# neuromodulation/py_neuromodulation

Hardware: AMD Instinct MI355X
Metric: windows/sec (all features), 256 ch @ 1 kHz (higher is better)
Workload: dtype f32; 1 GPU; 256ch/GPU @1kHz, W=1000, hop=100, 1024 hops/step, all 9 hot-path features, 4 bands, notch50+CAR, z-score normalisation; channels_per_gpu=256, features_per_window=9984, parallelism=channel-shard x1, no collective

## Files before the change

py_neuromodulation_amd/csrc/nmx_k_bank_w64.h:

```cpp
#pragma once

#include "nmx_k_bank.h"
#include "nmx_k_fft500.h"
#include "nmx_k_sharpwave.h"

#ifdef NMX_HOST_EMU
#define NMX_UNROLL
#else
#define NMX_UNROLL _Pragma("unroll")
#endif

#ifdef NMX_HOST_EMU
#define NMX_SCHED_FENCE() ((void)0)
#else
#define NMX_SCHED_FENCE() __builtin_amdgcn_sched_barrier(0)
#endif

#if defined(NMX_BANK_PROFILE) && !defined(NMX_HOST_EMU)
#define NMX_PROF_DECL long long pf_t = clock64(), pf_acc[8] = {0, 0, 0, 0, 0, 0, 0, 0};
#define NMX_PROF(i) { const long long t_ = clock64(); pf_acc[i] += t_ - pf_t; pf_t = t_; }
#define NMX_PROF_PRINT(w, c)                                                                                          \
  if ((w) == 5 && ((c) == 3 || (c) == 40) && (threadIdx.x & 63) == 0)                                                  \
    printf("bank profile w=%d c=%d: load+fwd %lld | spectral+passA %lld | passB load+dft %lld | passB store %lld | "  \
           "passC %lld | variance %lld | series stores %lld | partners %lld (cycles, whole item, %d filters)\n", (w), (c), pf_acc[0],   \
// ... 417 lines not shown
      }
#endif
    }
  }
  NMX_WSYNC();
  NMX_LANE_LOOP { nmx_w64_passA<-1>(v[NMX_LI], X, l); }
  NMX_WSYNC();
  NMX_LANE_LOOP { nmx_w64_passB_load_lds<-1, TAB>(v[NMX_LI], X, twB, l); }
  NMX_WSYNC();
  NMX_LANE_LOOP { nmx_w64_passB_store(v[NMX_LI], X, l); }
  NMX_WSYNC();
  NMX_LANE_LOOP {
    nmx_c2* vv = v[NMX_LI];
    nmx_w64_passC_lds<-1, TAB>(vv, X, twC, l);
    NMX_UNROLL
    for (int i = 0; i < 16; ++i) zr[NMX_LI][i] = vv[i];
  }
  NMX_WSYNC();
  NMX_PROF(0)

#ifndef NMX_HOST_EMU
  nmx_c2 zcr[16];
  if (PAD == 0) {
    const int l = (int)(threadIdx.x & 63);
    NMX_UNROLL
    for (int r = 0; r < 16; ++r) {
      const nmx_c2 zs = zr[0][NMX_J2I(15 - r)];
      nmx_c2 zc = nmx_mk2(__shfl(zs.x, (64 - l) & 63), __shfl(zs.y, (64 - l) & 63));
      if (l == 0) zc = (r == 0) ? zr[0][0] : zr[0][NMX_J2I((16 - r) & 15)];
      zcr[r] = zc;
    }
  }
#endif
  NMX_PROF(6)
  const int yoff = (PAD == 1) ? A.pad_half : 0;
  for (int fi = 0; fi < A.n_filters; ++fi) {
    const NmxFilterDev& F = A.f[fi];
    const float* NMX_RESTRICT Hs = TAB ? tab + (size_t)fi * 2 * NMX_W64_N : AA.Hs[fi];
    const float* NMX_RESTRICT Hd = TAB ? tab + (size_t)fi * 2 * NMX_W64_N + NMX_W64_N : AA.Hd[fi];
    NMX_LANE_LOOP {
      nmx_c2* vv = v[NMX_LI];
      NMX_UNROLL
      for (int r = 0; r < 16; ++r) {
        const nmx_c2 zk = zr[NMX_LI][NMX_J2I(r)];
#ifdef NMX_HOST_EMU
        nmx_c2 zc = zr[(64 - l) & 63][NMX_J2I(15 - r)];
        if (l == 0) zc = (r == 0) ? zr[NMX_LI][0] : zr[NMX_LI][NMX_J2I((16 - r) & 15)];
#else
        nmx_c2 zc;
        if (PAD == 0) {
          zc = zcr[r];
        } else {
          const nmx_c2 zs = zr[0][NMX_J2I(15 - r)];
          zc = nmx_mk2(__shfl(zs.x, (64 - l) & 63), __shfl(zs.y, (64 - l) & 63));
          if (l == 0) zc = (r == 0) ? zr[0][0] : zr[0][NMX_J2I((16 - r) & 15)];
        }
#endif
        const float ha = (Hs + l)[64 * r], hb = (Hd + l)[64 * r];
        vv[r] = nmx_c2_axpby_swap(ha, zk, hb, zc);
        if ((r & 3) == 3) NMX_SCHED_FENCE();
      }
      nmx_w64_passA<+1>(vv, X, l);
    }
    NMX_WSYNC();
    NMX_PROF(1)
    NMX_LANE_LOOP { nmx_w64_passB_load_lds<+1, TAB>(v[NMX_LI], X, twB, l); }
    NMX_WSYNC();
    NMX_PROF(2)
    NMX_LANE_LOOP { nmx_w64_passB_store(v[NMX_LI], X, l); }
    NMX_WSYNC();
    NMX_PROF(3)
    NMX_LANE_LOOP { nmx_w64_passC_lds<+1, TAB>(v[NMX_LI], X, twC, l); }
    NMX_PROF(4)

    if (F.bp_seglen > 0) {
      const bool need_mc = MC && (A.bp_features & 6u) != 0;
      if (!need_mc) {
        const int lo = W - F.bp_seglen + yoff, hi = W + yoff;
        float part[NMX_LANES], part2[NMX_LANES];
        NMX_LANE_LOOP {
          nmx_c2 acc = nmx_mk2(0.f, 0.f), acc2 = nmx_mk2(0.f, 0.f);
#if defined(NMX_HOST_EMU)
          NMX_UNROLL
          for (int i = 0; i < 16; ++i) {
            const int mb = 64 * (i >> 2) + 256 * (i & 3);
            if (2 * mb + 127 < lo || 2 * mb >= hi) continue;
            nmx_c2 val = v[NMX_LI][i];
            if (!(2 * mb >= lo && 2 * mb + 127 < hi)) val = nmx_w64_range_mask(val, l + mb, lo, hi);
            acc = nmx_cadd(acc, val);
            acc2 = nmx_c2_fma(val, val, acc2);
          }
#else
          const unsigned span = (unsigned)(hi - lo);
          const int s_l = 2 * l - lo;
          NMX_UNROLL
          for (int i = 0; i < 16; ++i) {
            const int sb = s_l + 2 * (64 * (i >> 2) + 256 * (i & 3));
            nmx_c2 val = v[NMX_LI][i];
            val.x = (unsigned)sb < span ? val.x : 0.f;
            val.y = (unsigned)(sb + 1) < span ? val.y : 0.f;
            acc = nmx_cadd(acc, val);
            acc2 = nmx_c2_fma(val, val, acc2);
          }
#endif
          part[NMX_LI] = acc.x + acc.y;
          part2[NMX_LI] = acc2.x + acc2.y;
        }
        float tot, tot2;
        NMX_W64_REDUCE_SUM(part, tot);
        NMX_W64_REDUCE_SUM(part2, tot2);
        const float mean = tot / (float)F.bp_seglen;
        tot = tot2 - mean * tot;
        if (mean * mean * (float)F.bp_seglen > 4.f * tot) {
          NMX_LANE_LOOP {
            nmx_c2 acc = nmx_mk2(0.f, 0.f);
            const nmx_c2 mean2 = nmx_mk2(mean, mean);
            NMX_UNROLL
            for (int i = 0; i < 16; ++i) {
              const int mb = 64 * (i >> 2) + 256 * (i & 3);
              if (2 * mb + 127 < lo || 2 * mb >= hi) continue;
              nmx_c2 d = nmx_csub(v[NMX_LI][i], mean2);
              if (!(2 * mb >= lo && 2 * mb + 127 < hi)) d = nmx_w64_range_mask(d, l + mb, lo, hi);
              acc = nmx_c2_fma(d, d, acc);
            }
            part[NMX_LI] = acc.x + acc.y;
          }
          NMX_W64_REDUCE_SUM(part, tot);
        }
        const float act = tot / (float)F.bp_seglen;
        NMX_LANE_LOOP {
          if (l == 0) {
            const int col = A.bp_cols.base + c * A.bp_cols.ch_stride + F.bp_band * A.bp_cols.a_stride;
            out_row[col] = nmx_bp_activity(A.bp_log ? log10f(act) : act, (A.bp_kalman_mask >> F.bp_band) & 1u);
          }
        }
      } else {
        NMX_WSYNC();
        NMX_LANE_LOOP {
          NMX_UNROLL
          for (int i = 0; i < 16; ++i) X[l + 64 * (i >> 2) + 256 * (i & 3)] = v[NMX_LI][i];
        }
        NMX_WSYNC();
        const float* y = (const float*)X + yoff;
        float act, mob, comp;
        nmx_hjorth(y + (W - F.bp_seglen), F.bp_seglen, red, 1, true, act, mob, comp);
        if (NMX_TID == 0) {
          int col = A.bp_cols.base + c * A.bp_cols.ch_stride + F.bp_band * A.bp_cols.a_stride;
          if (A.bp_features & 1u) { out_row[col] = nmx_bp_activity(A.bp_log ? log10f(act) : act, (A.bp_kalman_mask >> F.bp_band) & 1u); col += A.bp_cols.b_stride; }
          if (A.bp_features & 2u) { out_row[col] = nmx_nan_to_num(mob); col += A.bp_cols.b_stride; }
          if (A.bp_features & 4u) out_row[col] = nmx_nan_to_num(comp);
        }
      }
    }
    NMX_PROF(5)
    if (PAD == 0) {
      float* dsw = F.sw_index >= 0
          ? A.sw_out + (((long long)w * A.n_channels + c) * A.n_sw_filters + F.sw_index) * W : nullptr;
      float* dyb = F.burst_index >= 0
          ? AA.yb_out + (((long long)w * A.n_channels + c) * A.n_burst_bands + F.burst_index) * W : nullptr;
#ifdef NMX_HOST_EMU
      NMX_LANE_LOOP {
        for (int i = 0; i < 16; ++i) {
          const int m = l + 64 * (i >> 2) + 256 * (i & 3);
          const nmx_c2 val = v[NMX_LI][i];
          if (2 * m < W) { if (dsw) dsw[2 * m] = val.x; if (dyb) dyb[2 * m] = val.x; }
          if (2 * m + 1 < W) { if (dsw) dsw[2 * m + 1] = val.y; if (dyb) dyb[2 * m + 1] = val.y; }
        }
      }
#else
      const int l = (int)(threadIdx.x & 63);
      for (int dst = 0; dst < 2; ++dst) {
        float* d = dst ? dyb : dsw;
        if (!d) continue;
        const nmx_rsrc rs = nmx_make_rsrc(d, 4 * W);
        if ((W & 1) == 0) {
          NMX_UNROLL
          for (int i = 0; i < 16; ++i) {
            __builtin_amdgcn_raw_buffer_store_b64(v[0][i], rs, 8 * l + 512 * (i >> 2) + 2048 * (i & 3), 0, NMX_SERIES_STORE_AUX);
          }
        } else {
          NMX_UNROLL
          for (int i = 0; i < 16; ++i) {
            const int off = 8 * l + 512 * (i >> 2) + 2048 * (i & 3);
            __builtin_amdgcn_raw_buffer_store_b32(__float_as_uint(v[0][i].x), rs, off, 0, NMX_SERIES_STORE_AUX);
            __builtin_amdgcn_raw_buffer_store_b32(__float_as_uint(v[0][i].y), rs, off + 4, 0, NMX_SERIES_STORE_AUX);
          }
        }
      }
#endif
    } else if (F.store_raw) {
#ifndef NMX_HOST_EMU
      {
        const int l = (int)(threadIdx.x & 63);
        const nmx_rsrc rd = nmx_make_rsrc(A.y_out + ((long long)w * A.n_channels + c) * W, 4 * W);
        NMX_UNROLL
        for (int i = 0; i < 16; ++i) {
          const int s0 = 2 * (l + 64 * (i >> 2) + 256 * (i & 3)) - yoff;
          nmx_c2 val = v[0][i];
          if (A.residual) {
            const nmx_rsrc rx = nmx_make_rsrc(src, 4 * W);
            nmx_c2 xw = nmx_mk2(__uint_as_float(__builtin_amdgcn_raw_buffer_load_b32(rx, 4 * s0, 0, 0)),
                                __uint_as_float(__builtin_amdgcn_raw_buffer_load_b32(rx, 4 * s0 + 4, 0, 0)));
            if (A.clean_on_load) xw = nmx_mk2(nmx_clean_bl(xw.x), nmx_clean_bl(xw.y));
            val = xw - val;
          }
          __builtin_amdgcn_raw_buffer_store_b32(__float_as_uint(val.x), rd, 4 * s0, 0, 0);
          __builtin_amdgcn_raw_buffer_store_b32(__float_as_uint(val.y), rd, 4 * s0 + 4, 0, 0);
        }
      }
#else
      float* d2 = A.y_out + ((long long)w * A.n_channels + c) * W - yoff;
      NMX_LANE_LOOP {
        NMX_UNROLL
        for (int i = 0; i < 16; ++i) {
          const int s0 = 2 * (l + 64 * (i >> 2) + 256 * (i & 3));
          const nmx_c2 val = v[NMX_LI][i];
          if (s0 >= yoff && s0 < W + yoff)
            d2[s0] = A.residual ? (A.clean_on_load ? nmx_clean(src[s0 - yoff]) : src[s0 - yoff]) - val.x : val.x;
          if (s0 + 1 >= yoff && s0 + 1 < W + yoff)
            d2[s0 + 1] = A.residual ? (A.clean_on_load ? nmx_clean(src[s0 + 1 - yoff]) : src[s0 + 1 - yoff]) - val.y : val.y;
        }
      }
#endif
    }
    NMX_WSYNC();
    NMX_PROF(7)
  }
  NMX_PROF_PRINT(w, c)
}

struct NmxHilbertArgs {
  const float* y;
  float* env;
  int W;
  NmxFft hil_r;
  NmxFft hil_c;
  int hil_full;
  int off_a, off_b, off_y, lds_floats;
  const float* w500_tab;
  const float* w1000_tab;
  const float* floor;
  unsigned char* full;
  int n_seq, overlap;
  int long_mode, split_d, sub_m;
  const float2* tw_n;
  int slab_floats;
  int slab_blocks;
  float* slab;
};

NMX_DEV void nmx_hilbert_long_item(const NmxHilbertArgs& A, long long item, float* smem, float* slab);

NMX_DEV void nmx_hilbert_item(const NmxHilbertArgs& A, long long item, float* smem) {
  if (A.long_mode) { nmx_hilbert_long_item(A, item, smem, A.slab); return; }
  float2* bufA = (float2*)(smem + A.off_a);
  float2* bufB = (float2*)(smem + A.off_b);
  const int W = A.W, Wh = W >> 1;
  const float* src = A.y + item * W;
  float* dst = A.env + item * W;
  if (!A.hil_full) {
    float* ys = smem + A.off_y;
    float* pk = (float*)bufB;
    nmx_stage_row(src, W, [=](int i, float v) { pk[i] = v; ys[i] = v; });
    NMX_SYNC();
    const float2* Zy = nmx_fft_auto<-1, true>(A.hil_r, bufB, bufA, bufB);
    float2* Yb = (Zy == bufA) ? bufB : bufA;
    for (int k = NMX_TID; k <= Wh; k += NMX_NT) Yb[k] = nmx_rfft_bin(Zy, A.hil_r.twr, Wh, k);
    NMX_SYNC();
    float2* Pre = (Yb == bufA) ? bufB : bufA;
    for (int k = NMX_TID; k < Wh; k += NMX_NT) {
      const float2 yk = Yb[k], yn = Yb[Wh - k];
      const float2 xk = k == 0 ? make_float2(0.f, 0.f) : make_float2(yk.y, -yk.x);
      const float2 xn = k == 0 ? make_float2(0.f, 0.f) : make_float2(yn.y, -yn.x);
      Pre[k] = nmx_irfft_pre(xk, xn, A.hil_r.twr[k]);
    }
    NMX_SYNC();
    const float* ht = (const float*)nmx_fft_auto<+1, true>(A.hil_r, Pre, Yb, Pre);
    const float invW = 1.f / (float)W;
    for (int i = NMX_TID; i < W; i += NMX_NT) {
      const float re = ys[i], im = ht[i] * invW;
      dst[i] = nmx_sqrt_fast(re * re + im * im);
    }
    return;
  }
  nmx_stage_row(src, W, [=](int i, float v) { bufB[i] = make_float2(v, 0.f); });
  NMX_SYNC();
  const float2* Zy = nmx_fft_auto<-1, true>(A.hil_r, bufB, bufA, bufB);
  float2* Ab = (Zy == bufA) ? bufB : bufA;
  const float invW = 1.f / (float)W;
  for (int k = NMX_TID; k < W; k += NMX_NT) {
    float2 val = make_float2(0.f, 0.f);
    if (k == 0) val = Zy[0];
    else if (k <= (W - 1) / 2) val = make_float2(2.f * Zy[k].x, 2.f * Zy[k].y);
    Ab[k] = make_float2(val.x * invW, val.y * invW);
  }
  NMX_SYNC();
  float2* Zbuf = (Ab == bufA) ? bufB : bufA;
  const float2* an = nmx_fft_auto<+1, true>(A.hil_c, Ab, Zbuf, Ab);
  for (int i = NMX_TID; i < W; i += NMX_NT) dst[i] = nmx_sqrt_fast(an[i].x * an[i].x + an[i].y * an[i].y);
}

#ifndef NMX_HOST_EMU
#define NMX_W500_LDS_FLOATS (1008 + 1000)
template <bool SPARSE>
NMX_DEV void nmx_hilbert_w500_item(const NmxHilbertArgs& A, long long item, float* smem) {
  const int l = NMX_TID;
  nmx_c2* hb = (nmx_c2*)smem;
  nmx_c2* ha = hb + 504;
#ifdef NMX_DEBUG_HILBERT_SAMEROW
  const nmx_rsrc rin = nmx_make_rsrc(A.y + (item & 1023) * 1000, 4000);
#else
  const nmx_rsrc rin = nmx_make_rsrc(A.y + item * 1000, 4000);
#endif
  const nmx_rsrc rout = nmx_make_rsrc(A.env + item * 1000, 4000);
  const float fl = SPARSE ? A.floor[(int)item % A.n_seq] : 0.f;
  NmxW500TwReg T;
  T.load(A.w500_tab, l);
  nmx_c2 y[8];
#pragma unroll
  for (int q = 0; q < 8; ++q) y[q] = __builtin_amdgcn_raw_buffer_load_b64(rin, 8 * l + 512 * q, 0, 0);
#pragma unroll
  for (int q = 0; q < 8; ++q)
    if (q < 7 || l < 52) hb[l + 64 * q] = y[q];
  NMX_WAVE_FENCE();
  const nmx_c2* ht = nmx_w500_hilbert(ha, hb, T, (const nmx_c2*)A.w500_tab + NMX_W500_TW_N, l);
  if (SPARSE) {
    bool hit = !(fl > -INFINITY);
#pragma unroll
    for (int q = 0; q < 8; ++q) {
      const nmx_c2 h = ht[l + 64 * q];
      y[q] = nmx_mk2(nmx_sqrt_fast(y[q].x * y[q].x + h.x * h.x), nmx_sqrt_fast(y[q].y * y[q].y + h.y * h.y));
      hit = hit || ((q < 7 || l < 52) && (y[q].x >= fl || y[q].y >= fl));
    }
    const bool row = __ballot(hit) != 0ull;
    const int keep = 1000 - A.overlap;
#pragma unroll
    for (int q = 0; q < 8; ++q)
      if (row || 2 * (l + 64 * q) + 2 > keep) __builtin_amdgcn_raw_buffer_store_b64(y[q], rout, 8 * l + 512 * q, 0, 0);
    if (l == 0) A.full[item] = row ? 1 : 0;
    return;
  }
#pragma unroll
  for (int q = 0; q < 8; ++q) {
    const nmx_c2 h = ht[l + 64 * q];
    const nmx_c2 e = nmx_mk2(nmx_sqrt_fast(y[q].x * y[q].x + h.x * h.x), nmx_sqrt_fast(y[q].y * y[q].y + h.y * h.y));
    __builtin_amdgcn_raw_buffer_store_b64(e, rout, 8 * l + 512 * q, 0, 0);
  }
}
#define NMX_W1000_LDS_FLOATS 2000
template <bool SPARSE>
NMX_DEV void nmx_hilbert_w1000_item(const NmxHilbertArgs& A, long long item, float* smem) {
  const int l = NMX_TID;
  nmx_c2* hb = (nmx_c2*)smem;
  nmx_c2* ha = hb;
  const nmx_rsrc rin = nmx_make_rsrc(A.y + item * 2000, 8000);
  const nmx_rsrc rout = nmx_make_rsrc(A.env + item * 2000, 8000);
  const float fl = SPARSE ? A.floor[(int)(item % (long long)A.n_seq)] : 0.f;
  NmxW1000TwReg T;
  T.load(A.w1000_tab, l);
  nmx_c2 y[16];
#pragma unroll
  for (int q = 0; q < 16; ++q) y[q] = __builtin_amdgcn_raw_buffer_load_b64(rin, 8 * l + 512 * q, 0, 0);
#pragma unroll
  for (int q = 0; q < 16; ++q)
    if (q < 15 || l < 40) hb[l + 64 * q] = y[q];
  NMX_WAVE_FENCE();
  const nmx_c2* ht = nmx_w1000_hilbert(ha, hb, T, (const nmx_c2*)A.w1000_tab + NMX_W1000_TW_N, l);
  if (SPARSE) {
    bool hit = !(fl > -INFINITY);
#pragma unroll
    for (int q = 0; q < 16; ++q) {
      if (!(q < 15 || l < 40)) continue;
      const nmx_c2 h = ht[l + 64 * q];
      y[q] = nmx_mk2(nmx_sqrt_fast(y[q].x * y[q].x + h.x * h.x), nmx_sqrt_fast(y[q].y * y[q].y + h.y * h.y));
      hit = hit || y[q].x >= fl || y[q].y >= fl;
    }
    const bool row = __ballot(hit) != 0ull;
    const int keep = 2000 - A.overlap;
#pragma unroll
    for (int q = 0; q < 16; ++q)
      if ((q < 15 || l < 40) && (row || 2 * (l + 64 * q) + 2 > keep))
        __builtin_amdgcn_raw_buffer_store_b64(y[q], rout, 8 * l + 512 * q, 0, 0);
    if (l == 0) A.full[item] = row ? 1 : 0;
    return;
  }
#pragma unroll
  for (int q = 0; q < 16; ++q) {
    if (!(q < 15 || l < 40)) continue;
    const nmx_c2 h = ht[l + 64 * q];
    const nmx_c2 e = nmx_mk2(nmx_sqrt_fast(y[q].x * y[q].x + h.x * h.x), nmx_sqrt_fast(y[q].y * y[q].y + h.y * h.y));
    __builtin_amdgcn_raw_buffer_store_b64(e, rout, 8 * l + 512 * q, 0, 0);
  }
}
#endif

#include "nmx_k_hilbert_long.h"
```

py_neuromodulation_amd/csrc/nmx_k_fft500.h:

```cpp
#pragma once

#include "nmx_device.h"

template <int DIR>
NMX_DEV nmx_c2 nmx_twd(nmx_c2 t) { return DIR > 0 ? nmx_mk2(t.x, -t.y) : t; }

#define NMX_W500_TW_N (17 * 64)
#define NMX_W500_CS_N 500
#define NMX_W500_TAB_FLOATS (2 * (NMX_W500_TW_N + NMX_W500_CS_N))

#ifndef NMX_HOST_EMU

struct NmxW500TwReg {
  nmx_c2 a[17];
  NMX_DEV void load(const float* tab, int lane) {
#pragma unroll
    for (int i = 0; i < 17; ++i) a[i] = ((const nmx_c2*)tab)[i * 64 + lane];
  }
  NMX_DEV nmx_c2 get(int i) const { return a[i]; }
};
struct NmxW500TwRegC {
  nmx_c2 a[9], b[2];
  NMX_DEV void load(const float* tab, int lane) {
#pragma unroll
    for (int i = 0; i < 9; ++i) a[i] = ((const nmx_c2*)tab)[i * 64 + lane];
    b[0] = ((const nmx_c2*)tab)[9 * 64 + lane];
    b[1] = ((const nmx_c2*)tab)[13 * 64 + lane];
  }
  NMX_DEV nmx_c2 get(int i) const {
    if (i < 9) return a[i];
    const nmx_c2 w1 = b[(i - 9) >> 2];
    const int r = (i - 9) & 3;
    if (r == 0) return w1;
    const nmx_c2 w2 = nmx_cmul(w1, w1);
    if (r == 1) return w2;
    if (r == 2) return nmx_cmul(w2, w1);
    return nmx_cmul(w2, w2);
  }
};
struct NmxW500TwLds {
  const nmx_c2* p;
  NMX_DEV nmx_c2 get(int i) const { return p[64 * i]; }
};

template <int DIR>
NMX_DEV void nmx_dft5_c2(nmx_c2& x0, nmx_c2& x1, nmx_c2& x2, nmx_c2& x3, nmx_c2& x4) {
  const float c1 = 0.30901699437494745f, c2 = -0.80901699437494745f;
  const float s1 = DIR * 0.95105651629515353f, s2 = DIR * 0.58778525229247314f;
  const nmx_c2 t1 = x1 + x4, t2 = x2 + x3, d1 = x1 - x4, d2 = x2 - x3;
  const nmx_c2 m1 = x0 + c1 * t1 + c2 * t2, m2 = x0 + c2 * t1 + c1 * t2;
  const nmx_c2 u1 = s1 * d1 + s2 * d2, u2 = s2 * d1 - s1 * d2;
  x0 = x0 + t1 + t2;
  x1 = nmx_add_ib<+1>(m1, u1); x4 = nmx_add_ib<-1>(m1, u1);
  x2 = nmx_add_ib<+1>(m2, u2); x3 = nmx_add_ib<-1>(m2, u2);
}

template <int DIR>
NMX_DEV void nmx_dft10_c2(nmx_c2* v) {
  nmx_c2 e0 = v[0], e1 = v[2], e2 = v[4], e3 = v[6], e4 = v[8];
  nmx_c2 o0 = v[1], o1 = v[3], o2 = v[5], o3 = v[7], o4 = v[9];
  nmx_dft5_c2<DIR>(e0, e1, e2, e3, e4);
  nmx_dft5_c2<DIR>(o0, o1, o2, o3, o4);
  const float sg = (float)DIR;
  o1 = nmx_cmul(o1, nmx_mk2(0.80901699437494745f, sg * 0.58778525229247314f));
  o2 = nmx_cmul(o2, nmx_mk2(0.30901699437494745f, sg * 0.95105651629515353f));
  o3 = nmx_cmul(o3, nmx_mk2(-0.30901699437494745f, sg * 0.95105651629515353f));
  o4 = nmx_cmul(o4, nmx_mk2(-0.80901699437494745f, sg * 0.58778525229247314f));
  v[0] = e0 + o0; v[1] = e1 + o1; v[2] = e2 + o2; v[3] = e3 + o3; v[4] = e4 + o4;
  v[5] = e0 - o0; v[6] = e1 - o1; v[7] = e2 - o2; v[8] = e3 - o3; v[9] = e4 - o4;
}

template <int DIR, typename TW>
NMX_DEV nmx_c2* nmx_w500_fft(const nmx_c2* in, nmx_c2* a, nmx_c2* b, const TW& T, int lane) {
  nmx_c2 v[10];
  if (lane < 50) {
    nmx_ds_read_seq<400, 0>(v, nmx_lds_addr(in + lane), std::make_integer_sequence<int, 10>{});
    nmx_lds_wait8(v); nmx_lds_tie2(v[8], v[9]);
    nmx_dft10_c2<DIR>(v);
    nmx_c2* o = a + 10 * lane;
#pragma unroll
    for (int r = 0; r < 10; ++r) o[r] = v[r];
  }
  NMX_WAVE_FENCE();
  if (lane < 50) {
    nmx_ds_read_seq<400, 0>(v, nmx_lds_addr(a + lane), std::make_integer_sequence<int, 10>{});
    nmx_lds_wait8(v); nmx_lds_tie2(v[8], v[9]);
#pragma unroll
    for (int r = 1; r < 10; ++r) v[r] = nmx_cmul_tw<(DIR > 0)>(v[r], T.get(r - 1));
    nmx_dft10_c2<DIR>(v);
    const int q = lane / 10, k = lane - 10 * q;
    nmx_c2* o = b + 100 * q + k;
#pragma unroll
    for (int r = 0; r < 10; ++r) o[10 * r] = v[r];
  }
  NMX_WAVE_FENCE();
  if (lane < 50) {
#pragma unroll
    for (int h = 0; h < 2; ++h) {
      nmx_c2 x[5];
      nmx_ds_read_seq<800, 0>(x, nmx_lds_addr(b + lane + 50 * h), std::make_integer_sequence<int, 5>{});
      nmx_lds_wait5(x[0], x[1], x[2], x[3], x[4]);
      nmx_c2 x0 = x[0], x1 = x[1], x2 = x[2], x3 = x[3], x4 = x[4];
      x1 = nmx_cmul_tw<(DIR > 0)>(x1, T.get(9 + 4 * h));
      x2 = nmx_cmul_tw<(DIR > 0)>(x2, T.get(10 + 4 * h));
      x3 = nmx_cmul_tw<(DIR > 0)>(x3, T.get(11 + 4 * h));
      x4 = nmx_cmul_tw<(DIR > 0)>(x4, T.get(12 + 4 * h));
      nmx_dft5_c2<DIR>(x0, x1, x2, x3, x4);
      nmx_c2* o = a + lane + 50 * h;
      o[0] = x0; o[100] = x1; o[200] = x2; o[300] = x3; o[400] = x4;
    }
  }
  NMX_WAVE_FENCE();
  return a;
}

template <typename TW>
NMX_DEV nmx_c2* nmx_w500_fft_fwd_low(const nmx_c2* in, nmx_c2* a, nmx_c2* b, const TW& T, int lane, int k_hi) {
  nmx_c2 v[10];
  if (lane < 50) {
    nmx_ds_read_seq<400, 0>(v, nmx_lds_addr(in + lane), std::make_integer_sequence<int, 10>{});
    nmx_lds_wait8(v); nmx_lds_tie2(v[8], v[9]);
    nmx_dft10_c2<-1>(v);
    nmx_c2* o = a + 10 * lane;
#pragma unroll
    for (int r = 0; r < 10; ++r) o[r] = v[r];
  }
  NMX_WAVE_FENCE();
  if (lane < 50) {
    nmx_ds_read_seq<400, 0>(v, nmx_lds_addr(a + lane), std::make_integer_sequence<int, 10>{});
    nmx_lds_wait8(v); nmx_lds_tie2(v[8], v[9]);
#pragma unroll
    for (int r = 1; r < 10; ++r) v[r] = nmx_cmul_tw<0>(v[r], T.get(r - 1));
    nmx_dft10_c2<-1>(v);
    const int q = lane / 10, k = lane - 10 * q;
    nmx_c2* o = b + 100 * q + k;
#pragma unroll
    for (int r = 0; r < 10; ++r) o[10 * r] = v[r];
  }
  NMX_WAVE_FENCE();
  if (lane < 50) {
    const float c1 = 0.30901699437494745f, c2 = -0.80901699437494745f;
    const float s1 = -0.95105651629515353f, s2 = -0.58778525229247314f;
#pragma unroll
    for (int h = 0; h < 2; ++h) {
      const int j = lane + 50 * h;
      const bool lo = j < k_hi, hi = j > 100 - k_hi;
      if (!(lo || hi)) continue;
      const nmx_c2* src = b + j;
      nmx_c2 x0 = src[0], x1 = src[100], x2 = src[200], x3 = src[300], x4 = src[400];
      x1 = nmx_cmul_tw<0>(x1, T.get(9 + 4 * h));
      x2 = nmx_cmul_tw<0>(x2, T.get(10 + 4 * h));
      x3 = nmx_cmul_tw<0>(x3, T.get(11 + 4 * h));
      x4 = nmx_cmul_tw<0>(x4, T.get(12 + 4 * h));
      const nmx_c2 t1 = x1 + x4, t2 = x2 + x3;
      if (lo) a[j] = x0 + t1 + t2;
      if (hi) {
        const nmx_c2 d1 = x1 - x4, d2 = x2 - x3;
        const nmx_c2 m1 = x0 + c1 * t1 + c2 * t2;
        const nmx_c2 u1 = s1 * d1 + s2 * d2;
        a[j + 400] = nmx_add_ib<-1>(m1, u1);
      }
    }
  }
  NMX_WAVE_FENCE();
  return a;
}

template <typename TW>
NMX_DEV const nmx_c2* nmx_w500_hilbert(nmx_c2* a, nmx_c2* b, const TW& T, const nmx_c2* cs, int lane) {
  const nmx_c2* Z = nmx_w500_fft<-1>(b, a, b, T, lane);
#pragma unroll
  for (int q = 0; q < 8; ++q) {
    const int k = lane + 64 * q;
    if (k < 500) {
      const nmx_c2 zk = Z[k], zc = Z[k == 0 ? 0 : 500 - k], w = cs[k];
      b[k] = nmx_mk2(w.x * zc.x - w.y * zk.y, w.y * zk.x - w.x * zc.y);
    }
  }
  NMX_WAVE_FENCE();
  return nmx_w500_fft<+1>(b, a, b, T, lane);
}

#define NMX_W1000_TW_N (27 * 64)
#define NMX_W1000_CS_N 1000
#define NMX_W1000_TAB_FLOATS (2 * (NMX_W1000_TW_N + NMX_W1000_CS_N))
struct NmxW1000TwReg {
  nmx_c2 a[27];
  NMX_DEV void load(const float* tab, int lane) {
#pragma unroll
    for (int i = 0; i < 27; ++i) a[i] = ((const nmx_c2*)tab)[i * 64 + lane];
  }
  NMX_DEV nmx_c2 get(int i) const { return a[i]; }
};

template <int DIR, typename TW>
NMX_DEV nmx_c2* nmx_w1000_fft(const nmx_c2* in, nmx_c2* a, nmx_c2* b, const TW& T, int lane) {
  nmx_c2 v[10], u[10];
  if (lane < 50) {
    nmx_ds_read_seq<800, 0>(v, nmx_lds_addr(in + lane), std::make_integer_sequence<int, 10>{});
    nmx_ds_read_seq<800, 0>(u, nmx_lds_addr(in + lane + 50), std::make_integer_sequence<int, 10>{});
    nmx_lds_wait8(v); nmx_lds_tie2(v[8], v[9]); nmx_lds_tie8(u); nmx_lds_tie2(u[8], u[9]);
    nmx_dft10_c2<DIR>(v);
    nmx_dft10_c2<DIR>(u);
  }
  NMX_WAVE_FENCE();
  if (lane < 50) {
    nmx_c2* o = a + 10 * lane;
#pragma unroll
    for (int r = 0; r < 10; ++r) { o[r] = v[r]; o[500 + r] = u[r]; }
  }
  NMX_WAVE_FENCE();
  if (lane < 50) {
    nmx_ds_read_seq<800, 0>(v, nmx_lds_addr(a + lane), std::make_integer_sequence<int, 10>{});
    nmx_ds_read_seq<800, 0>(u, nmx_lds_addr(a + lane + 50), std::make_integer_sequence<int, 10>{});
    nmx_lds_wait8(v); nmx_lds_tie2(v[8], v[9]); nmx_lds_tie8(u); nmx_lds_tie2(u[8], u[9]);
#pragma unroll
    for (int r = 1; r < 10; ++r) { v[r] = nmx_cmul_tw<(DIR > 0)>(v[r], T.get(r - 1)); u[r] = nmx_cmul_tw<(DIR > 0)>(u[r], T.get(r - 1)); }
    nmx_dft10_c2<DIR>(v);
    nmx_dft10_c2<DIR>(u);
  }
  NMX_WAVE_FENCE();
  if (lane < 50) {
    const int q0 = lane / 10, k = lane - 10 * q0;
    nmx_c2* o = b + 100 * q0 + k;
#pragma unroll
    for (int r = 0; r < 10; ++r) { o[10 * r] = v[r]; o[500 + 10 * r] = u[r]; }
  }
  NMX_WAVE_FENCE();
  if (lane < 50) {
    nmx_ds_read_seq<800, 0>(v, nmx_lds_addr(b + lane), std::make_integer_sequence<int, 10>{});
    nmx_ds_read_seq<800, 0>(u, nmx_lds_addr(b + lane + 50), std::make_integer_sequence<int, 10>{});
    nmx_lds_wait8(v); nmx_lds_tie2(v[8], v[9]); nmx_lds_tie8(u); nmx_lds_tie2(u[8], u[9]);
#pragma unroll
    for (int r = 1; r < 10; ++r) { v[r] = nmx_cmul_tw<(DIR > 0)>(v[r], T.get(9 + r - 1)); u[r] = nmx_cmul_tw<(DIR > 0)>(u[r], T.get(18 + r - 1)); }
    nmx_dft10_c2<DIR>(v);
    nmx_dft10_c2<DIR>(u);
  }
  NMX_WAVE_FENCE();
  if (lane < 50) {
    nmx_c2* o = a + lane;
#pragma unroll
    for (int r = 0; r < 10; ++r) { o[100 * r] = v[r]; o[50 + 100 * r] = u[r]; }
  }
  NMX_WAVE_FENCE();
  return a;
}

template <typename TW>
NMX_DEV const nmx_c2* nmx_w1000_hilbert(nmx_c2* a, nmx_c2* b, const TW& T, const nmx_c2* cs, int lane) {
  const nmx_c2* Z = nmx_w1000_fft<-1>(b, a, b, T, lane);
  nmx_c2 zp[16];
#pragma unroll
  for (int q = 0; q < 16; ++q) {
    const int k = lane + 64 * q;
    zp[q] = nmx_mk2(0.f, 0.f);
    if (k < 1000) {
      const nmx_c2 zk = Z[k], zc = Z[k == 0 ? 0 : 1000 - k], w = cs[k];
      zp[q] = nmx_mk2(w.x * zc.x - w.y * zk.y, w.y * zk.x - w.x * zc.y);
    }
  }
  NMX_WAVE_FENCE();
#pragma unroll
  for (int q = 0; q < 16; ++q)
    if (lane + 64 * q < 1000) b[lane + 64 * q] = zp[q];
  NMX_WAVE_FENCE();
  return nmx_w1000_fft<+1>(b, a, b, T, lane);
}
#endif
```

py_neuromodulation_amd/csrc/nmx_wave.hip:

```cpp
#ifndef NMX_NT_FIXED
#error "compile with -DNMX_NT_FIXED=64"
#endif
#include <hip/hip_runtime.h>
#include <cstdio>
#include <cstdlib>

#include "nmx_k_bursts.h"
#include "nmx_k_bank_w64.h"
#include "nmx_k_burst_stat_reg.h"
#include "nmx_k_scan.h"
#include "nmx_k_td.h"
#include "nmx_k_timeosc_w1000.h"
#include "nmx_k_timeosc_w510.h"
#include "nmx_k_sharpwave.h"

extern __shared__ __attribute__((aligned(16))) float nmx_smem_wave[];

static int waves_per_wg(size_t lds_one, int dflt = 1) {
  const char* v = getenv("NMX_WAVES_PER_WG");
  const int k = (v && atoi(v) >= 1 && atoi(v) <= 4) ? atoi(v) : 0;
  int kk = k ? k : dflt;
  while (kk > 1 && lds_one * kk > 64 * 1024) --kk;
  return kk;
}
#define NMX_WAVE_ITEM(item, smem, n_items, slice)                                                   \
  const int wave_ = __builtin_amdgcn_readfirstlane((int)(threadIdx.x >> 6));                        \
  const int item = (int)blockIdx.x * (int)(blockDim.x >> 6) + wave_;                                \
  if (item >= (n_items)) return;                                                                    \
  float* smem = nmx_smem_wave + wave_ * (slice)

__global__ void __launch_bounds__(256) nmx_kern_burst_stat(const NmxBurstStatArgs A, int n_items, int slice) {
  const int wave = __builtin_amdgcn_readfirstlane((int)(threadIdx.x >> 6));
  const int item = blockIdx.x * (blockDim.x >> 6) + wave;
  if (item >= n_items) return;
  const int bi = item % A.n_bands, r = item / A.n_bands;
  nmx_burst_stat_item(A, r / A.n_channels, r % A.n_channels, bi, nmx_smem_wave + wave * slice);
}

template <int CH, bool SPARSE = false>
__global__ void __launch_bounds__(256) nmx_kern_burst_stat_reg(const NmxBurstStatArgs A, int n_items) {
  const int wave = __builtin_amdgcn_readfirstlane((int)(threadIdx.x >> 6));
  const int item = blockIdx.x * 4 + wave;
  if (item >= n_items) return;
  const int bi = item % A.n_bands, r = item / A.n_bands;
  nmx_burst_stat_item_reg<CH, SPARSE>(A, r / A.n_channels, r % A.n_channels, bi);
}

__global__ void __launch_bounds__(256) nmx_kern_burst_stat_scan(const NmxBurstStatArgs A, int n_items) {
  const int wave = __builtin_amdgcn_readfirstlane((int)(threadIdx.x >> 6));
  const int item = blockIdx.x * 4 + wave;
  if (item >= n_items) return;
  const int bi = item % A.n_bands, r = item / A.n_bands;
  nmx_burst_stat_scan_item(A, r / A.n_channels, r % A.n_channels, bi, nmx_smem_wave + wave * A.lds_floats);
}

__global__ void __launch_bounds__(256) nmx_kern_sharp(const NmxSharpArgs A, int n_items, int slice) {
  const int wave = __builtin_amdgcn_readfirstlane((int)(threadIdx.x >> 6));
  const int item = blockIdx.x * (blockDim.x >> 6) + wave;
  if (item >= n_items) return;
  const int fi = item % A.n_filters, r = item / A.n_filters;
  nmx_sharp_item(A, r / A.n_channels, r % A.n_channels, fi, nmx_smem_wave + wave * slice);
}

template <int NR, bool LL>
__global__ void __launch_bounds__(64) nmx_kern_burst_thr_wave(const NmxBurstThrArgs A) {
  __builtin_amdgcn_s_setprio(3);
  const int item = blockIdx.x;
  nmx_burst_thr_wave_item<NR, LL>(A, item / A.n_bands, item % A.n_bands, nmx_smem_wave);
}

extern "C" void nmx_wave_launch_burst_thr(const NmxBurstThrArgs* A, int n_items, int nr, bool list_lds, size_t lds, hipStream_t s) {
  if (nr == 2 && list_lds) NMX_LAUNCH((nmx_kern_burst_thr_wave<2, true>), dim3(n_items), dim3(64), lds, s, *A);
  else if (nr != 2) NMX_LAUNCH((nmx_kern_burst_thr_wave<4, false>), dim3(n_items), dim3(64), lds, s, *A);
  else NMX_LAUNCH((nmx_kern_burst_thr_wave<2, false>), dim3(n_items), dim3(64), lds, s, *A);
}

__global__ void __launch_bounds__(256) nmx_kern_hilbert_w500(const NmxHilbertArgs A, int n_items) {
  NMX_WAVE_ITEM(item, smem, n_items, NMX_W500_LDS_FLOATS);
  nmx_hilbert_w500_item<false>(A, (long long)item, smem);
}
__global__ void __launch_bounds__(256) nmx_kern_hilbert_w500_sparse(const NmxHilbertArgs A, int n_items) {
  NMX_WAVE_ITEM(item, smem, n_items, NMX_W500_LDS_FLOATS);
  nmx_hilbert_w500_item<true>(A, (long long)item, smem);
}

extern "C" void nmx_wave_launch_hilbert_w500(const NmxHilbertArgs* A, long long n_items, hipStream_t s) {
  const int k = waves_per_wg((size_t)NMX_W500_LDS_FLOATS * 4);
  const dim3 grid((unsigned)((n_items + k - 1) / k)), block(64 * k);
  if (A->full) NMX_LAUNCH(nmx_kern_hilbert_w500_sparse, grid, block, (size_t)NMX_W500_LDS_FLOATS * 4 * k, s, *A, (int)n_items);
  else NMX_LAUNCH(nmx_kern_hilbert_w500, grid, block, (size_t)NMX_W500_LDS_FLOATS * 4 * k, s, *A, (int)n_items);
}

__global__ void __launch_bounds__(256) nmx_kern_hilbert_w1000(const NmxHilbertArgs A, long long n_items) {
  const int wave = __builtin_amdgcn_readfirstlane((int)(threadIdx.x >> 6));
  const long long item = (long long)blockIdx.x * 4 + wave;
  if (item >= n_items) return;
  nmx_hilbert_w1000_item<false>(A, item, nmx_smem_wave + wave * NMX_W1000_LDS_FLOATS);
}
__global__ void __launch_bounds__(256) nmx_kern_hilbert_w1000_sparse(const NmxHilbertArgs A, long long n_items) {
  const int wave = __builtin_amdgcn_readfirstlane((int)(threadIdx.x >> 6));
  const long long item = (long long)blockIdx.x * 4 + wave;
  if (item >= n_items) return;
  nmx_hilbert_w1000_item<true>(A, item, nmx_smem_wave + wave * NMX_W1000_LDS_FLOATS);
}

extern "C" void nmx_wave_launch_hilbert_w1000(const NmxHilbertArgs* A, long long n_items, hipStream_t s) {
  const dim3 grid((unsigned)((n_items + 3) / 4));
  if (A->full) NMX_LAUNCH(nmx_kern_hilbert_w1000_sparse, grid, dim3(256), (size_t)4 * NMX_W1000_LDS_FLOATS * 4, s, *A, n_items);
  else NMX_LAUNCH(nmx_kern_hilbert_w1000, grid, dim3(256), (size_t)4 * NMX_W1000_LDS_FLOATS * 4, s, *A, n_items);
}

template <int NB, unsigned SPEC = 0>
__global__ void __launch_bounds__(256) nmx_kern_timeosc_w1000(const NmxTimeOscArgs A, int n_items, int slice) {
  NMX_WAVE_ITEM(item, smem, n_items, slice);
  const int w = nmx_uniform_i(item / A.n_channels), c = nmx_uniform_i(item % A.n_channels);
  NmxW500TwReg T;
  T.load(A.w500_tab, (int)(threadIdx.x & 63));
  NmxTdRegs R;
  nmx_td_load<1000>(A, w, c, R);
  nmx_timeosc_w1000_body<NB, false, NmxW500TwReg, false, SPEC>(A, w, c, R, T, smem);
}

template <int NB, unsigned SPEC = 0>
__global__ void __launch_bounds__(64) __attribute__((amdgpu_waves_per_eu(3, 4)))
nmx_kern_timeosc_w1000_low(const NmxTimeOscArgs A0, int n_items) {
  typedef const NmxTimeOscArgs __attribute__((address_space(4)))* nmx_karg_p;
  nmx_karg_p Ap = (nmx_karg_p)__builtin_amdgcn_kernarg_segment_ptr();
  const NmxTimeOscArgs& A = *(const NmxTimeOscArgs*)Ap;
  const int lane = (int)(threadIdx.x & 63);
  NmxW500TwReg T;
  T.load(A.w500_tab, lane);
  {
    const float2* twr = (A.fft.enabled ? A.fft : A.welch).fft.twr;
    float2* twl = (float2*)(nmx_smem_wave + NMX_TOW_LOW_TWL_OFF);
    twl[lane] = twr[lane];
    if (lane < 38) twl[64 + lane] = twr[64 + lane];
  }
  const int C = A.n_channels, step = (int)gridDim.x;
  int item = (int)blockIdx.x;
  if (item >= n_items) return;
  NmxTdRegs R;
  nmx_f4 Xn[4];
  int w = nmx_uniform_i(item / C), c = nmx_uniform_i(item - w * C);
  nmx_td_load_x<1000>(A, w, c, R);
  NMX_WAVE_FENCE();
#pragma nounroll
  for (;;) {
    const int nxt = item + step;
    int wn = 0, cn = 0;
    nmx_td_rest_from_x<1000>(R);
    {
      const int pf = nxt < n_items ? nxt : item;
      wn = nmx_uniform_i(pf / C); cn = nmx_uniform_i(pf - wn * C);
      NmxTdRegs Rn;
      nmx_td_load_x<1000>(A, wn, cn, Rn);
      Xn[0] = Rn.x[0]; Xn[1] = Rn.x[1]; Xn[2] = Rn.x[2]; Xn[3] = Rn.x[3];
    }
    asm volatile("" : "+s"(Ap));
    nmx_timeosc_w1000_body<NB, true, NmxW500TwReg, false, SPEC>(*(const NmxTimeOscArgs*)Ap, w, c, R, T, nmx_smem_wave);
    NMX_WAVE_FENCE();
    if (nxt >= n_items) break;
    item = nxt; w = wn; c = cn;
    R.x[0] = Xn[0]; R.x[1] = Xn[1]; R.x[2] = Xn[2]; R.x[3] = Xn[3];
  }
}


extern "C" void nmx_wave_launch_timeosc_w1000_low(const NmxTimeOscArgs* A, int n_items, int n_cu, hipStream_t s) {
  int grid = n_cu * 12;
  const int C = A->n_channels;
  if (grid > C && grid % C) grid -= grid % C;
  if (grid > n_items) grid = n_items;
  const size_t lds = (size_t)NMX_TOW_LOW_LDS_FLOATS * 4;
  const unsigned spec = nmx_tow_spec(*A);
  static_assert(NMX_TOW_SPEC_C2 == 65809u && NMX_TOW_SPEC_DEFAULT == 196915u && NMX_TOW_SPEC_ALL == 196923u, "reported kernel names");
  if (A->n_bands <= 4 && spec == NMX_TOW_SPEC_C2)
    NMX_LAUNCH_AS("nmx_kern_timeosc_w1000_low<4, 65809u>", (nmx_kern_timeosc_w1000_low<4, NMX_TOW_SPEC_C2>), dim3(grid), dim3(64), lds, s, *A, n_items);
  else if (A->n_bands <= 4 && spec == NMX_TOW_SPEC_DEFAULT)
    NMX_LAUNCH_AS("nmx_kern_timeosc_w1000_low<4, 196915u>", (nmx_kern_timeosc_w1000_low<4, NMX_TOW_SPEC_DEFAULT>), dim3(grid), dim3(64), lds, s, *A, n_items);
  else if (A->n_bands <= 4) NMX_LAUNCH(nmx_kern_timeosc_w1000_low<4>, dim3(grid), dim3(64), lds, s, *A, n_items);
  else NMX_LAUNCH(nmx_kern_timeosc_w1000_low<8>, dim3(grid), dim3(64), lds, s, *A, n_items);
}

extern "C" void nmx_wave_launch_timeosc_w1000(const NmxTimeOscArgs* A, int n_items, hipStream_t s) {
  const size_t lds = (size_t)(A->stft.enabled ? NMX_TOW_LDS_FLOATS : NMX_TOW_LDS_FLOATS_NOSTFT) * 4;
  const int k = waves_per_wg(lds);
  const dim3 grid((unsigned)((n_items + k - 1) / k)), block(64 * k);
  const int slice = (int)(lds / 4);
  if (A->n_bands <= 4 && nmx_tow_spec(*A) == NMX_TOW_SPEC_ALL)
    NMX_LAUNCH_AS("nmx_kern_timeosc_w1000<4, 196923u>", (nmx_kern_timeosc_w1000<4, NMX_TOW_SPEC_ALL>), grid, block, lds * k, s, *A, n_items, slice);
  else if (A->n_bands <= 4) NMX_LAUNCH(nmx_kern_timeosc_w1000<4>, grid, block, lds * k, s, *A, n_items, slice);
  else NMX_LAUNCH(nmx_kern_timeosc_w1000<8>, grid, block, lds * k, s, *A, n_items, slice);
}

template <int NB>
__global__ void __launch_bounds__(64) nmx_kern_timeosc_w1000_todo(const NmxTimeOscArgs A, int n_items) {
  const int lane = (int)(threadIdx.x & 63);
  const int C = A.n_channels, n_windows = n_items / C, n_tiles = ((n_windows + 15) / 16) * C;
  NmxW500TwReg T;
  bool loaded = false;
  for (int base = (int)blockIdx.x * 64; base < n_tiles; base += (int)gridDim.x * 64) {
    const int i = base + lane;
    const unsigned mine = i < n_tiles ? A.todo[i] : 0u;
    unsigned long long m = __ballot(mine != 0u);
    while (m) {
      const int src = (int)__ffsll((long long)m) - 1;
      m &= m - 1;
      const int tile = base + src;
      unsigned bits = (unsigned)__builtin_amdgcn_readlane((int)mine, src);
      const int g = tile / C, c = nmx_uniform_i(tile - g * C);
      while (bits) {
        const int j = __ffs((int)bits) - 1;
        bits &= bits - 1;
        if (!loaded) { T.load(A.w500_tab, lane); loaded = true; }
        const int w = nmx_uniform_i(16 * g + j);
        NmxTdRegs R;
        nmx_td_load<1000>(A, w, c, R);
        nmx_timeosc_w1000_body<NB, false, NmxW500TwReg, false, 0>(A, w, c, R, T, nmx_smem_wave);
        NMX_WAVE_FENCE();
      }
    }
  }
}
extern "C" void nmx_wave_launch_timeosc_w1000_todo(const NmxTimeOscArgs* A, int n_items, hipStream_t s) {
  const size_t lds = (size_t)NMX_TOW_LDS_FLOATS_NOSTFT * 4;
  const int n_windows = n_items / A->n_channels, n_tiles = ((n_windows + 15) / 16) * A->n_channels;
  const int blocks = (n_tiles + 63) / 64;
  const int grid = blocks < 256 * 8 ? blocks : 256 * 8;
  if (A->n_bands <= 4) NMX_LAUNCH_AS("nmx_kern_timeosc_w1000_todo", nmx_kern_timeosc_w1000_todo<4>, dim3(grid), dim3(64), lds, s, *A, n_items);
  else NMX_LAUNCH_AS("nmx_kern_timeosc_w1000_todo", nmx_kern_timeosc_w1000_todo<8>, dim3(grid), dim3(64), lds, s, *A, n_items);
}

template <int NB>
__global__ void __launch_bounds__(256) nmx_kern_timeosc_stft500(const NmxTimeOscArgs A, int n_items) {
  NMX_WAVE_ITEM(item, smem, n_items, NMX_TOS_LDS_FLOATS);
  nmx_timeosc_stft500_item<NB>(A, item / A.n_channels, item % A.n_channels, smem);
}
extern "C" void nmx_wave_launch_timeosc_stft500(const NmxTimeOscArgs* A, int n_items, hipStream_t s) {
  const int k = waves_per_wg((size_t)NMX_TOS_LDS_FLOATS * 4);
  const dim3 grid((unsigned)((n_items + k - 1) / k)), block(64 * k);
  if (A->n_bands <= 4) NMX_LAUNCH(nmx_kern_timeosc_stft500<4>, grid, block, (size_t)NMX_TOS_LDS_FLOATS * 4 * k, s, *A, n_items);
  else NMX_LAUNCH(nmx_kern_timeosc_stft500<8>, grid, block, (size_t)NMX_TOS_LDS_FLOATS * 4 * k, s, *A, n_items);
}

#ifndef NMX_W510_WAVES
#define NMX_W510_WAVES 4
#endif
#if NMX_W510_WAVES
#define NMX_W510_WPE __attribute__((amdgpu_waves_per_eu(NMX_W510_WAVES, NMX_W510_WAVES)))
#else
#define NMX_W510_WPE
#endif
template <int NB>
__global__ void __launch_bounds__(256) NMX_W510_WPE nmx_kern_timeosc_w510(const NmxTimeOscArgs A0, int n_items, int slice) {
  NMX_WAVE_ITEM(item, smem, n_items, slice);
  typedef const NmxTimeOscArgs __attribute__((address_space(4)))* nmx_karg_p;
  const NmxTimeOscArgs& A = *(const NmxTimeOscArgs*)(nmx_karg_p)__builtin_amdgcn_kernarg_segment_ptr();
  nmx_timeosc_w510_item<NB>(A, A.w510_tab, item / A.n_channels, item % A.n_channels, smem);
}
extern "C" void nmx_wave_launch_timeosc_w510(const NmxTimeOscArgs* A, int n_items, hipStream_t s) {
  const int slice = NMX_TO510_LDS_FLOATS(A->W);
  const int k = waves_per_wg((size_t)slice * 4);
  const dim3 grid((unsigned)((n_items + k - 1) / k)), block(64 * k);
  if (A->n_bands <= 4) NMX_LAUNCH(nmx_kern_timeosc_w510<4>, grid, block, (size_t)slice * 4 * k, s, *A, n_items, slice);
  else NMX_LAUNCH(nmx_kern_timeosc_w510<8>, grid, block, (size_t)slice * 4 * k, s, *A, n_items, slice);
}

__global__ void __launch_bounds__(256) nmx_kern_scan(const NmxTimeOscArgs A, int n_items, int n_windows, int order) {
  const int wave = __builtin_amdgcn_readfirstlane((int)(threadIdx.x >> 6));
  const int item = blockIdx.x * 4 + wave;
  if (item >= n_items) return;
  if (order) nmx_td_item(A, item % n_windows, item / n_windows);
  else nmx_td_item(A, item / A.n_channels, item % A.n_channels);
}

extern "C" void nmx_wave_launch_scan(const NmxTimeOscArgs* A, int n_items, hipStream_t s) {
  const int order = 0;
  NMX_LAUNCH(nmx_kern_scan, dim3((n_items + 3) / 4), dim3(256), 0, s, *A, n_items, n_items / A->n_channels, order);
}

__global__ void __launch_bounds__(256) nmx_kern_sharp_dense(const NmxSharpArgs A, int n_items, int slice) {
  NMX_WAVE_ITEM(item, smem, n_items, slice);
  const int fi = item % A.n_filters, r = item / A.n_filters;
  nmx_sharp_item_dense(A, r / A.n_channels, r % A.n_channels, fi, (long long)item, smem);
}

extern "C" void nmx_wave_launch_sharp_dense(const NmxSharpArgs* A, int n_items, hipStream_t s) {
  const int slice = (A->dz_lds_floats + 3) & ~3;
  const int k = waves_per_wg((size_t)slice * 4, 2);
  NMX_LAUNCH(nmx_kern_sharp_dense, dim3((unsigned)((n_items + k - 1) / k)), dim3(64 * k), (size_t)slice * 4 * k, s, *A, n_items, slice);
}

__global__ void __launch_bounds__(64) nmx_kern_sharp_todo(const NmxSharpArgs A, int n_items, const unsigned char* todo) {
  const int lane = (int)(threadIdx.x & 63);
  for (int base = (int)blockIdx.x * 64; base < n_items; base += (int)gridDim.x * 64) {
    const int i = base + lane;
    unsigned long long m = __ballot(i < n_items && todo[i] != 0);
    while (m) {
      const int item = base + (int)__ffsll((long long)m) - 1;
      m &= m - 1;
      const int fi = item % A.n_filters, r = item / A.n_filters;
      nmx_sharp_item(A, r / A.n_channels, r % A.n_channels, fi, nmx_smem_wave);
      NMX_SYNC();
    }
  }
}

extern "C" void nmx_wave_launch_sharp_todo(const NmxSharpArgs* A, int n_items, size_t lds, const unsigned char* todo,
                                           hipStream_t s) {
  const int blocks = (n_items + 63) / 64;
  const int grid = blocks < 256 * 14 ? blocks : 256 * 14;
  NMX_LAUNCH(nmx_kern_sharp_todo, dim3(grid), dim3(64), lds, s, *A, n_items, todo);
}

extern "C" void nmx_wave_launch_burst_stat(const NmxBurstStatArgs* A, NmxBurstStatKind kind, int n_items, size_t lds, hipStream_t s) {
  const dim3 grid4((n_items + 3) / 4);
  switch (kind) {
    case NMX_BSTAT_REG16_SPARSE: NMX_LAUNCH_AS("nmx_kern_burst_stat_reg_sparse<16>", (nmx_kern_burst_stat_reg<16, true>), grid4, dim3(256), 0, s, *A, n_items); return;
    case NMX_BSTAT_REG16: NMX_LAUNCH(nmx_kern_burst_stat_reg<16>, grid4, dim3(256), 0, s, *A, n_items); return;
    case NMX_BSTAT_REG32_SPARSE: NMX_LAUNCH_AS("nmx_kern_burst_stat_reg_sparse<32>", (nmx_kern_burst_stat_reg<32, true>), grid4, dim3(256), 0, s, *A, n_items); return;
    case NMX_BSTAT_REG32: NMX_LAUNCH(nmx_kern_burst_stat_reg<32>, grid4, dim3(256), 0, s, *A, n_items); return;
    case NMX_BSTAT_SCAN: NMX_LAUNCH(nmx_kern_burst_stat_scan, grid4, dim3(256), (size_t)A->lds_floats * 4 * 4, s, *A, n_items); return;
    case NMX_BSTAT_GENERIC: break;
  }
  const int k = waves_per_wg(lds);
  const int slice = (int)((lds / 4 + 3) & ~(size_t)3);
  NMX_LAUNCH(nmx_kern_burst_stat, dim3((n_items + k - 1) / k), dim3(64 * k), (size_t)slice * 4 * k, s, *A, n_items, slice);
}

extern "C" void nmx_wave_launch_sharp(const NmxSharpArgs* A, int n_items, size_t lds, hipStream_t s) {
  const int k = waves_per_wg(lds, 2);
  const int slice = (int)((lds / 4 + 3) & ~(size_t)3);
  NMX_LAUNCH(nmx_kern_sharp, dim3((n_items + k - 1) / k), dim3(64 * k), (size_t)slice * 4 * k, s, *A, n_items, slice);
}
```

Baseline: 170,700 windows/s.

## Make W500 Hilbert kernel persistent with next-row prefetch and register-held coefficients

Turns the W500 Hilbert envelope kernel into a persistent grid-stride loop sized from the CU count (8 waves per CU by default). Each wave loads twiddles and the Hilbert cs coefficients into registers once and prefetches the next row's input while it works on the current row. This removes the per-item launch and table-load overhead and hides global load latency. It adds register pressure (waves_per_eu pinned to 4), and the sparse path now writes out-of-range stores to a dummy offset instead of branching.

Result: no change. 170,700 windows/s, median of 2 (+0.0%).

```diff
diff --git a/py_neuromodulation_amd/csrc/nmx_k_bank_w64.h b/py_neuromodulation_amd/csrc/nmx_k_bank_w64.h
--- a/py_neuromodulation_amd/csrc/nmx_k_bank_w64.h
+++ b/py_neuromodulation_amd/csrc/nmx_k_bank_w64.h
@@ -743,51 +743,90 @@
 
 #ifndef NMX_HOST_EMU
 #define NMX_W500_LDS_FLOATS (1008 + 1000)
+#ifndef NMX_HIL_W500_CSREG
+#define NMX_HIL_W500_CSREG 1
+#endif
+#ifndef NMX_HIL_W500_PREFETCH
+#define NMX_HIL_W500_PREFETCH 1
+#endif
+#ifdef NMX_DEBUG_HILBERT_SAMEROW
+#define NMX_HIL_W500_SRC(i) (A.y + (long long)((i) & 1023) * 1000)
+#else
+#define NMX_HIL_W500_SRC(i) (A.y + (long long)(i) * 1000)
+#endif
+NMX_DEV void nmx_hilbert_w500_load(const NmxHilbertArgs& A, int item, int l, nmx_c2* y) {
+  const nmx_rsrc rin = nmx_make_rsrc(NMX_HIL_W500_SRC(item), 4000);
+#pragma unroll
+  for (int q = 0; q < 8; ++q) y[q] = __builtin_amdgcn_raw_buffer_load_b64(rin, 8 * l + 512 * q, 0, 0);
+}
+NMX_DEV void nmx_hilbert_w500_stage(nmx_c2* hb, int l, const nmx_c2* y) {
+#pragma unroll
+  for (int q = 0; q < 8; ++q)
+    if (q < 7 || l < 52) hb[l + 64 * q] = y[q];
+}
 template <bool SPARSE>
-NMX_DEV void nmx_hilbert_w500_item(const NmxHilbertArgs& A, long long item, float* smem) {
+NMX_DEV void nmx_hilbert_w500_rows(const NmxHilbertArgs& A, int first, int step, int n_items, float* smem) {
   const int l = NMX_TID;
   nmx_c2* hb = (nmx_c2*)smem;
   nmx_c2* ha = hb + 504;
-#ifdef NMX_DEBUG_HILBERT_SAMEROW
-  const nmx_rsrc rin = nmx_make_rsrc(A.y + (item & 1023) * 1000, 4000);
-#else
-  const nmx_rsrc rin = nmx_make_rsrc(A.y + item * 1000, 4000);
-#endif
-  const nmx_rsrc rout = nmx_make_rsrc(A.env + item * 1000, 4000);
-  const float fl = SPARSE ? A.floor[(int)item % A.n_seq] : 0.f;
   NmxW500TwReg T;
   T.load(A.w500_tab, l);
+#if NMX_HIL_W500_CSREG
+  NmxW500CsReg cs;
+  cs.load((const nmx_c2*)A.w500_tab + NMX_W500_TW_N, l);
+#else
+  const NmxW500CsMem cs{(const nmx_c2*)A.w500_tab + NMX_W500_TW_N};
+#endif
   nmx_c2 y[8];
-#pragma unroll
-  for (int q = 0; q < 8; ++q) y[q] = __builtin_amdgcn_raw_buffer_load_b64(rin, 8 * l + 512 * q, 0, 0);
-#pragma unroll
-  for (int q = 0; q < 8; ++q)
-    if (q < 7 || l < 52) hb[l + 64 * q] = y[q];
-  NMX_WAVE_FENCE();
-  const nmx_c2* ht = nmx_w500_hilbert(ha, hb, T, (const nmx_c2*)A.w500_tab + NMX_W500_TW_N, l);
-  if (SPARSE) {
-    bool hit = !(fl > -INFINITY);
-#pragma unroll
-    for (int q = 0; q < 8; ++q) {
-      const nmx_c2 h = ht[l + 64 * q];
-      y[q] = nmx_mk2(nmx_sqrt_fast(y[q].x * y[q].x + h.x * h.x), nmx_sqrt_fast(y[q].y * y[q].y + h.y * h.y));
-      hit = hit || ((q < 7 || l < 52) && (y[q].x >= fl || y[q].y >= fl));
-    }
-    const bool row = __ballot(hit) != 0ull;
-    const int keep = 1000 - A.overlap;
-#pragma unroll
-    for (int q = 0; q < 8; ++q)
-      if (row || 2 * (l + 64 * q) + 2 > keep) __builtin_amdgcn_raw_buffer_store_b64(y[q], rout, 8 * l + 512 * q, 0, 0);
-    if (l == 0) A.full[item] = row ? 1 : 0;
-    return;
-  }
-#pragma unroll
-  for (int q = 0; q < 8; ++q) {
-    const nmx_c2 h = ht[l + 64 * q];
-    const nmx_c2 e = nmx_mk2(nmx_sqrt_fast(y[q].x * y[q].x + h.x * h.x), nmx_sqrt_fast(y[q].y * y[q].y + h.y * h.y));
-    __builtin_amdgcn_raw_buffer_store_b64(e, rout, 8 * l + 512 * q, 0, 0);
-  }
-}
+  int item = first;
+  nmx_hilbert_w500_load(A, item, l, y);
+  nmx_hilbert_w500_stage(hb, l, y);
+#pragma nounroll
+  for (;;) {
+    const int nxt = item + step;
+    const nmx_rsrc rout = nmx_make_rsrc(A.env + (long long)item * 1000, 4000);
+    const float fl = SPARSE ? A.floor[item % A.n_seq] : 0.f;
+    NMX_WAVE_FENCE();
+    const nmx_c2* ht = nmx_w500_hilbert_cs(ha, hb, T, cs, l);
+#if NMX_HIL_W500_PREFETCH
+    nmx_c2 yn[8];
+    nmx_hilbert_w500_load(A, nxt < n_items ? nxt : item, l, yn);
+#endif
+    if (SPARSE) {
+      bool hit = !(fl > -INFINITY);
+#pragma unroll
+      for (int q = 0; q < 8; ++q) {
+        const nmx_c2 h = ht[l + 64 * q];
+        y[q] = nmx_mk2(nmx_sqrt_fast(y[q].x * y[q].x + h.x * h.x), nmx_sqrt_fast(y[q].y * y[q].y + h.y * h.y));
+        hit = hit || ((q < 7 || l < 52) && (y[q].x >= fl || y[q].y >= fl));
+      }
+      const bool row = __ballot(hit) != 0ull;
+      const int keep = 1000 - A.overlap;
+#pragma unroll
+      for (int q = 0; q < 8; ++q)
+        __builtin_amdgcn_raw_buffer_store_b64(y[q], rout, (row || 2 * (l + 64 * q) + 2 > keep) ? 8 * l + 512 * q : 4096, 0, 0);
+      __builtin_amdgcn_raw_buffer_store_b8((unsigned char)(row ? 1 : 0), nmx_make_rsrc(A.full + item, 1), l, 0, 0);
+    } else {
+#pragma unroll
+      for (int q = 0; q < 8; ++q) {
+        const nmx_c2 h = ht[l + 64 * q];
+        const nmx_c2 e = nmx_mk2(nmx_sqrt_fast(y[q].x * y[q].x + h.x * h.x), nmx_sqrt_fast(y[q].y * y[q].y + h.y * h.y));
+        __builtin_amdgcn_raw_buffer_store_b64(e, rout, 8 * l + 512 * q, 0, 0);
+      }
+    }
+    if (nxt >= n_items) break;
+    NMX_WAVE_FENCE();
+    item = nxt;
+#if NMX_HIL_W500_PREFETCH
+#pragma unroll
+    for (int q = 0; q < 8; ++q) y[q] = yn[q];
+#else
+    nmx_hilbert_w500_load(A, item, l, y);
+#endif
+    nmx_hilbert_w500_stage(hb, l, y);
+  }
+}
+#undef NMX_HIL_W500_SRC
 #define NMX_W1000_LDS_FLOATS 2000
 template <bool SPARSE>
 NMX_DEV void nmx_hilbert_w1000_item(const NmxHilbertArgs& A, long long item, float* smem) {
diff --git a/py_neuromodulation_amd/csrc/nmx_k_fft500.h b/py_neuromodulation_amd/csrc/nmx_k_fft500.h
--- a/py_neuromodulation_amd/csrc/nmx_k_fft500.h
+++ b/py_neuromodulation_amd/csrc/nmx_k_fft500.h
@@ -166,19 +166,35 @@
   return a;
 }
 
-template <typename TW>
-NMX_DEV const nmx_c2* nmx_w500_hilbert(nmx_c2* a, nmx_c2* b, const TW& T, const nmx_c2* cs, int lane) {
+struct NmxW500CsMem {
+  const nmx_c2* p;
+  NMX_DEV nmx_c2 get(int q, int k) const { (void)q; return p[k]; }
+};
+struct NmxW500CsReg {
+  nmx_c2 a[8];
+  NMX_DEV void load(const nmx_c2* cs, int lane) {
+#pragma unroll
+    for (int q = 0; q < 8; ++q) a[q] = cs[lane + 64 * q < 500 ? lane + 64 * q : 499];
+  }
+  NMX_DEV nmx_c2 get(int q, int k) const { (void)k; return a[q]; }
+};
+template <typename TW, typename CS>
+NMX_DEV const nmx_c2* nmx_w500_hilbert_cs(nmx_c2* a, nmx_c2* b, const TW& T, const CS& cs, int lane) {
   const nmx_c2* Z = nmx_w500_fft<-1>(b, a, b, T, lane);
 #pragma unroll
   for (int q = 0; q < 8; ++q) {
     const int k = lane + 64 * q;
     if (k < 500) {
-      const nmx_c2 zk = Z[k], zc = Z[k == 0 ? 0 : 500 - k], w = cs[k];
+      const nmx_c2 zk = Z[k], zc = Z[k == 0 ? 0 : 500 - k], w = cs.get(q, k);
       b[k] = nmx_mk2(w.x * zc.x - w.y * zk.y, w.y * zk.x - w.x * zc.y);
     }
   }
   NMX_WAVE_FENCE();
   return nmx_w500_fft<+1>(b, a, b, T, lane);
+}
+template <typename TW>
+NMX_DEV const nmx_c2* nmx_w500_hilbert(nmx_c2* a, nmx_c2* b, const TW& T, const nmx_c2* cs, int lane) {
+  return nmx_w500_hilbert_cs(a, b, T, NmxW500CsMem{cs}, lane);
 }
 
 #define NMX_W1000_TW_N (27 * 64)
diff --git a/py_neuromodulation_amd/csrc/nmx_wave.hip b/py_neuromodulation_amd/csrc/nmx_wave.hip
--- a/py_neuromodulation_amd/csrc/nmx_wave.hip
+++ b/py_neuromodulation_amd/csrc/nmx_wave.hip
@@ -75,18 +75,40 @@
   else NMX_LAUNCH((nmx_kern_burst_thr_wave<2, false>), dim3(n_items), dim3(64), lds, s, *A);
 }
 
-__global__ void __launch_bounds__(256) nmx_kern_hilbert_w500(const NmxHilbertArgs A, int n_items) {
+__global__ void __launch_bounds__(256) __attribute__((amdgpu_waves_per_eu(4, 4))) nmx_kern_hilbert_w500(const NmxHilbertArgs A, int n_items) {
   NMX_WAVE_ITEM(item, smem, n_items, NMX_W500_LDS_FLOATS);
-  nmx_hilbert_w500_item<false>(A, (long long)item, smem);
-}
-__global__ void __launch_bounds__(256) nmx_kern_hilbert_w500_sparse(const NmxHilbertArgs A, int n_items) {
+  nmx_hilbert_w500_rows<false>(A, item, (int)(gridDim.x * (blockDim.x >> 6)), n_items, smem);
+}
+__global__ void __launch_bounds__(256) __attribute__((amdgpu_waves_per_eu(4, 4))) nmx_kern_hilbert_w500_sparse(const NmxHilbertArgs A, int n_items) {
   NMX_WAVE_ITEM(item, smem, n_items, NMX_W500_LDS_FLOATS);
-  nmx_hilbert_w500_item<true>(A, (long long)item, smem);
-}
-
+  nmx_hilbert_w500_rows<true>(A, item, (int)(gridDim.x * (blockDim.x >> 6)), n_items, smem);
+}
+
+static int wave_cu_count() {
+  static std::atomic<int> seen[16];
+  int dev = 0, n = 0;
+  if (hipGetDevice(&dev) != hipSuccess || dev < 0 || dev >= 16) return 256;
+  if ((n = seen[dev].load(std::memory_order_relaxed)) > 0) return n;
+  if (hipDeviceGetAttribute(&n, hipDeviceAttributeMultiprocessorCount, dev) != hipSuccess || n <= 0) n = 256;
+  seen[dev].store(n, std::memory_order_relaxed);
+  return n;
+}
+
+#ifndef NMX_HIL_W500_WAVES_PER_CU
+#define NMX_HIL_W500_WAVES_PER_CU 8
+#endif
 extern "C" void nmx_wave_launch_hilbert_w500(const NmxHilbertArgs* A, long long n_items, hipStream_t s) {
   const int k = waves_per_wg((size_t)NMX_W500_LDS_FLOATS * 4);
-  const dim3 grid((unsigned)((n_items + k - 1) / k)), block(64 * k);
+  long long waves = n_items;
+  const char* v = getenv("NMX_HILBERT_RESIDENT");
+  if (!(v && atoi(v) == 0)) {
+    const long long held = (long long)wave_cu_count() * 16;
+    const char* g = getenv("NMX_HILBERT_GRID");
+    long long slots = g && atoi(g) >= 1 ? atoi(g) : (long long)wave_cu_count() * NMX_HIL_W500_WAVES_PER_CU;
+    if (slots > held) slots = held;
+    if (waves > slots) waves = slots;
+  }
+  const dim3 grid((unsigned)((waves + k - 1) / k)), block(64 * k);
   if (A->full) NMX_LAUNCH(nmx_kern_hilbert_w500_sparse, grid, block, (size_t)NMX_W500_LDS_FLOATS * 4 * k, s, *A, (int)n_items);
   else NMX_LAUNCH(nmx_kern_hilbert_w500, grid, block, (size_t)NMX_W500_LDS_FLOATS * 4 * k, s, *A, (int)n_items);
 }
```
